# tuneinsight/lattigo

Measured on AMD Instinct MI355X. Metric: ciphertext-mul+relin ops/s, higher is better.
Workload: dtype u64; 1 GPU; BGV logN=15, 12 Q-limbs [55,45x11] + 3 P-limbs [55x3], T=65537: ct x ct MulRelin (tensor + gadget product + ModDown), inputs resident in HBM; batch_per_gpu=256, logN=15, L=12, alpha=3, beta=4, parallelism=1 independent replicas, ciphertext-sharded

## Files before the change

### lattigo_amd/csrc/kernels.hip

```cpp
#include "kernels.h"

#include <atomic>
#include <cstdio>
#include <cstdlib>
#include <type_traits>
#include <mutex>
#include <unordered_map>
#include <vector>

namespace he {

namespace {
struct ProfRec { int id; hipEvent_t e0, e1; double bytes; };
struct ProfState { std::vector<ProfRec> recs; };
std::mutex g_prof_mu;
std::atomic<int> g_prof_active{0};
std::unordered_map<hipStream_t, ProfState> g_prof;
std::vector<hipEvent_t> g_prof_pool;
hipEvent_t prof_event_locked() {
    if (!g_prof_pool.empty()) { hipEvent_t e = g_prof_pool.back(); g_prof_pool.pop_back(); return e; }
    hipEvent_t e;
    (void)hipEventCreate(&e);
    return e;
}
// ... 177 lines not shown
    const uint64_t *tw;
    const double *twd;
    int N;
    int a;
    int flags;
    int scale;
    LimbTab tab;
    int epi;
    const uint64_t *epi_y, *epi_w;
    size_t epi_y_bs, epi_w_bs;
    uint64_t epi_s[kMaxLimbs];
    int zsplit;
    int epi2;
    uint64_t *out2;
    size_t out2_bs;
    const uint64_t *epi_y2, *epi_w2;
    size_t epi_y2_bs, epi_w2_bs;
    int epi_tensor;
    const uint64_t *ta0, *ta1, *tb0, *tb1;
    size_t ta0_bs, ta1_bs, tb0_bs, tb1_bs;
    uint64_t epi_ts[kMaxLimbs];
    uint64_t io_s[kMaxLimbs];
    int epi_y_f64;
    int epi_y_reduce;
    int nbatch, iters;
    int nbatch_prof = 0;
    int tprod = 0;
    unsigned sc_ginv = 0;
    int sc_logN = 0;
    const size_t *in_tab = nullptr;
    int cb = 0;
    const size_t *out_tab = nullptr, *out2_tab = nullptr, *epi_w_tab = nullptr, *epi_w2_tab = nullptr;
    const size_t *ta0_tab = nullptr, *ta1_tab = nullptr, *tb0_tab = nullptr, *tb1_tab = nullptr;
    const size_t *epi_y_tab = nullptr, *epi_y2_tab = nullptr;
};

__device__ __forceinline__ int lds_phys(int e) { return e + (e >> 4); }

__device__ __forceinline__ void wave_lds_sync() {
    __builtin_amdgcn_fence(__ATOMIC_RELEASE, "wavefront");
    __builtin_amdgcn_wave_barrier();
    __builtin_amdgcn_fence(__ATOMIC_ACQUIRE, "wavefront");
}
__device__ __forceinline__ void rows_sync(int sh) {
    if (sh <= 6) wave_lds_sync();
    else __syncthreads();
}
template <int T>
__device__ __forceinline__ int nat_e(int k, int tau) {
    constexpr int CH = T >= 64 ? 64 : T;
    return (tau / CH) * (16 * CH) + k * CH + (tau % CH);
}

int ntt_row_bits(int n) {
    return n <= 12 ? n : (n <= 15 ? 12 : 13);
}

template <int G4, bool INV, bool NC>
__device__ __forceinline__ void rows_round(uint64_t (&x)[16], const uint64_t *__restrict__ tw, int rowtw, int s0, int hi0,
                                           int tau, int sh, uint64_t q, uint64_t twoq, uint64_t qinv, const ModConst &mc,
                                           bool scale_last) {
    constexpr int g = G4, G = 1 << g, W = 16 / G;
    if constexpr (!INV) {
#pragma unroll
        for (int u = 0; u < g; u++) {
            const int d = 1 << (g - 1 - u);
#pragma unroll
            for (int w = 0; w < W; w++) {
                const int hi = (W == 1) ? hi0 : ((tau * W + w) >> sh);
                const int base = (rowtw << (s0 + u)) + (hi << u);
#pragma unroll
                for (int k = 0; k < G; k++) {
                    if (k & d) continue;
                    const uint64_t wv = tw[base + (k >> (g - u))];
                    if constexpr (NC) bfly_fwd_nc<true>(x[w * G + k], x[w * G + k + d], wv, q, qinv);
                    else bfly_fwd<true>(x[w * G + k], x[w * G + k + d], wv, q, twoq, qinv);
                }
            }
        }
    } else {
#pragma unroll
        for (int u = g - 1; u >= 0; u--) {
            const int d = 1 << (g - 1 - u);
            const bool last = scale_last && u == 0;
#pragma unroll
            for (int w = 0; w < W; w++) {
                const int hi = (W == 1) ? hi0 : ((tau * W + w) >> sh);
                const int base = (rowtw << (s0 + u)) + (hi << u);
#pragma unroll
                for (int k = 0; k < G; k++) {
                    if (k & d) continue;
                    const uint64_t wv = tw[base + (k >> (g - u))];
                    if (last) bfly_inv_scaled(x[w * G + k], x[w * G + k + d], mred(wv, mc.ninv, q, qinv), mc.ninv, q, twoq, qinv);
                    else bfly_inv(x[w * G + k], x[w * G + k + d], wv, q, twoq, qinv);
                }
            }
        }
    }
}

__device__ __forceinline__ void rows_tw16(uint64_t (&t)[15], const uint64_t *__restrict__ tw, int rowtw, int s0, int hi0) {
#pragma unroll
    for (int u = 0; u < 4; u++) {
        const int base = (rowtw << (s0 + u)) + (hi0 << u);
#pragma unroll
        for (int j = 0; j < (1 << u); j++) t[(1 << u) - 1 + j] = tw[base + j];
// ... 760 lines not shown
template <int LOGB>
__device__ __forceinline__ void mac_final_xfer(double (&x)[16], double *lds, int tau, bool store) {
    if constexpr (LOGB % 4 == 0) rows_lds_xfer_f64<LOGB, 4>(x, lds, tau, LOGB - 4, 0, store);
    else rows_lds_xfer_f64<LOGB, LOGB % 4>(x, lds, tau, LOGB - LOGB % 4, 0, store);
}
typedef __attribute__((address_space(3))) void *he_lds_ptr;
__device__ __forceinline__ unsigned lds_byte_addr(const void *p) { return (unsigned)(uintptr_t)(he_lds_ptr)p; }
__device__ __forceinline__ void glds16(const void *gsrc, unsigned lds_dst) {
    unsigned keep;
    asm volatile("s_mov_b32 %0, m0\n\ts_mov_b32 m0, %2\n\ts_nop 0\n\tglobal_load_lds_dwordx4 %1, off nt\n\ts_mov_b32 m0, %0"
                 : "=&s"(keep) : "v"(gsrc), "s"(lds_dst) : "memory");
}
struct MacEpiK {
    const uint64_t *ext; size_t ext_bs;
    uint64_t *out0, *out1; size_t out0_bs, out1_bs;
    const uint64_t *w0, *w1; size_t w0_bs, w1_bs;
    const uint64_t *ta0, *ta1, *tb0, *tb1; size_t ta0_bs, ta1_bs, tb0_bs, tb1_bs;
    int ext_f64, tensor, has_w0, has_w1;
    double sp[kMaxLimbs], tsp[kMaxLimbs];
    const size_t *etab;
    unsigned etab_rows;
    unsigned sc_ginv;
    int sc_logN;
    int gs_accum;
};
enum { ME_OUT0 = 0, ME_OUT1, ME_W0, ME_W1, ME_TA0, ME_TA1, ME_TB0, ME_TB1 };
__device__ __forceinline__ size_t meoff(const MacEpiK &e, int which, size_t bs, size_t z, unsigned nbatch) {
    const unsigned row = (e.etab_rows >> (4 * which)) & 0xFu;
    return (e.etab && row != 0xFu) ? (size_t)ldc(reinterpret_cast<const uint64_t *>(e.etab), (size_t)row * nbatch + z) : z * bs;
}
struct NttMacDmaArgs {
    NttMacKArgs k;
    MacEpiK e;
    unsigned nbatch, nitems;
    uint64_t limb_info[kMaxLimbs];
};
#ifdef HE_MAC_STAMPS
#ifndef HE_MAC_STAMP_ITEM
#define HE_MAC_STAMP_ITEM 10
#endif
#define MAC_STAMP2(i) do { __builtin_amdgcn_sched_barrier(0); if (t_cur == HE_MAC_STAMP_ITEM && g < 512u && (threadIdx.x & 63u) == 0) g_mac_stamps[((g * 4 + (threadIdx.x >> 6)) * 64) + (i)] = __builtin_amdgcn_s_memtime(); __builtin_amdgcn_sched_barrier(0); } while (0)
#else
#define MAC_STAMP2(i) do {} while (0)
#endif
template <int LOGB, bool QF64, bool EPI = false, bool SCAT = false, bool TEN = false>
__global__ void __launch_bounds__((1 << LOGB) / 16, 2) ntt_mac_f64_dma_kernel(NttMacDmaArgs AA) {
    static_assert(LOGB == 12 || LOGB == 13, "production row sizes only");
    constexpr int N2 = 1 << LOGB;
    constexpr int T = N2 / 16;
    constexpr int GREM = LOGB % 4;
    const NttMacKArgs &A = AA.k;
    __shared__ double lds[N2 + N2 / 16];
    __shared__ double pbuf[N2];
    __shared__ double tw1s[16 * 15];

    const unsigned tau = threadIdx.x, lane = tau & 63u;
    const unsigned wv = (unsigned)__builtin_amdgcn_readfirstlane((int)(tau >> 6));
    const unsigned G = gridDim.x, g = blockIdx.x;
    const bool xcd = ((G | AA.nitems) & 7u) == 0;
    const unsigned span = xcd ? AA.nitems >> 3 : AA.nitems, stride = xcd ? G >> 3 : G;
    const unsigned first = xcd ? g >> 3 : g, base = xcd ? (g & 7u) * span : 0u;
    auto item_of = [&](unsigned t) -> unsigned { const unsigned i = first + t * stride; return i < span ? base + i : ~0u; };

    struct Item {
        size_t bz, rowoff;
        int ql, rowtw, out_limb, mi, l;
        bool isP;
        double q, qi;
        const double *tw, *kbase;
    };
    auto decode = [&](unsigned w) -> Item {
        Item it;
        it.bz = w % AA.nbatch;
        const int l = (int)((w / AA.nbatch) % (unsigned)A.m.nlimbs);
        const int row = (int)(w / (AA.nbatch * (unsigned)A.m.nlimbs));
        const uint64_t info = AA.limb_info[l];
        it.l = l;
        const int mi = (int)(info & 0xff);
        it.mi = mi;
        const uint64_t *mcw = reinterpret_cast<const uint64_t *>(A.mc + mi);
        it.q = (double)ldc(mcw, 0); it.qi = __longlong_as_double((long long)ldc(mcw, 8));
        it.tw = A.twd + (size_t)mi * A.N;
        it.rowtw = (1 << A.a) + row;
        it.rowoff = (size_t)row * N2;
        it.kbase = A.keyd + (size_t)((info >> 8) & 0xff) * A.N + it.rowoff;
        it.ql = (int)((info >> 16) & 0xff);
        it.out_limb = (int)((info >> 24) & 0xff);
        it.isP = ((info >> 32) & 0xff) != 0;
        return it;
    };
    auto own_digit = [&](const Item &it, int d) -> bool {
        return A.m.own_alpha > 0 && !it.isP && it.ql >= d * A.m.own_alpha && it.ql < (d + 1) * A.m.own_alpha;
    };
    const int nd = A.m.beta + (EPI ? 2 : 0);
    auto digit_src = [&](const Item &it, int d) -> const uint64_t * {
        if (EPI && d >= A.m.beta)
            return AA.e.ext + ((size_t)(d - A.m.beta) * AA.nbatch + it.bz) * AA.e.ext_bs + (size_t)it.ql * A.N + it.rowoff;
        return own_digit(it, d) ? A.own + voff(A.own_tab, A.own_bs, it.bz) + (size_t)it.ql * A.N + it.rowoff
                                : A.dec + it.bz * A.dec_bs + (size_t)d * A.m.dec_dstride + (size_t)it.ql * A.N + it.rowoff;
    };
    const unsigned pw_addr = lds_byte_addr(pbuf) + wv * 8192u;
    auto dma_digit = [&](const uint64_t *src, unsigned lane) {
        const uint64_t *gp = src + ((lane >> 5) * T + 64u * wv + 2u * (lane & 31u));
#pragma unroll
        for (int j = 0; j < 8; j++) glds16(gp + (size_t)j * 2 * T, pw_addr + (unsigned)j * 1024u);
    };

    unsigned t = 0;
    unsigned w = item_of(0);
    if (w == ~0u) return;
    Item cur = decode(w);
    dma_digit(digit_src(cur, 0), lane);
    for (;;) {
        const unsigned t_cur = t; (void)t_cur;
        MAC_STAMP2(0);
        double acc0[16], acc1[16];
#pragma unroll
        for (int k = 0; k < 16; k++) { acc0[k] = 0.0; acc1[k] = 0.0; }
        const double q = cur.q, qi = cur.qi;
        if (tau < 240u) {
            const unsigned hi = tau / 15u, idx = tau - hi * 15u, u = 31u - (unsigned)__builtin_clz(idx + 1u), j = idx + 1u - (1u << u);
            tw1s[tau] = cur.tw[((unsigned)cur.rowtw << (4 + u)) + (hi << u) + j];
        }
        bool more = false;
        auto round0 = [&](double (&x)[16]) {
            double t0[15];
#pragma unroll
            for (int u = 0; u < 4; u++)
#pragma unroll
                for (int j = 0; j < (1 << u); j++) t0[(1 << u) - 1 + j] = ldcd(cur.tw, (size_t)(((unsigned)cur.rowtw << u) + j));
            rows_round16_f64<false>(x, t0, q, qi);
        };
        auto round1 = [&](double (&x)[16], unsigned tau) {
            rows_lds_xfer_f64<LOGB, 4>(x, lds, tau, 4, LOGB - 8, false);
            {
                double t1[15];
                const double *tp = tw1s + (tau >> (LOGB - 8)) * 15u;
#pragma unroll
                for (int i = 0; i < 15; i++) t1[i] = tp[i];
                rows_round16_f64<false>(x, t1, q, qi);
            }
            rows_lds_xfer_f64<LOGB, 4>(x, lds, tau, 4, LOGB - 8, true);
            rows_sync(LOGB - 8);
            rows_lds_xfer_f64<LOGB, 4>(x, lds, tau, 8, LOGB - 12, false);
        };
        auto transform = [&](int nk, double (&x)[16], unsigned tau, unsigned lane, const uint64_t *nsrc, const double *k0p,
                             const double *k1p, double (&kk0)[16], double (&kk1)[16]) {
            double t2[15];
            rows_tw16_f64(t2, cur.tw, cur.rowtw, 8, tau >> (LOGB - 12));
            __builtin_amdgcn_sched_barrier(0);
            asm volatile("s_waitcnt lgkmcnt(0)" ::: "memory");
            if (nsrc) dma_digit(nsrc, lane);
            __builtin_amdgcn_sched_barrier(0);
            round0(x);
            __syncthreads();
            rows_lds_xfer_f64<LOGB, 4>(x, lds, tau, 0, LOGB - 4, true);
            __syncthreads();
            round1(x, tau);
            __builtin_amdgcn_sched_barrier(0);
            if (nk >= 1) {
#pragma unroll
                for (int k = 0; k < 16; k++) kk0[k] = k0p[(unsigned)(k * T)];
            }
            __builtin_amdgcn_sched_barrier(0);
            rows_round16_f64<false>(x, t2, q, qi);
            __builtin_amdgcn_sched_barrier(0);
            if (nk >= 2) {
#pragma unroll
                for (int k = 0; k < 16; k++) kk1[k] = k1p[(unsigned)(k * T)];
            }
            __builtin_amdgcn_sched_barrier(0);
            if constexpr (GREM > 0) {
                rows_lds_xfer_f64<LOGB, 4>(x, lds, tau, 8, LOGB - 12, true);
                rows_sync(LOGB - 12);
                rows_lds_xfer_f64<LOGB, GREM>(x, lds, tau, 12, 0, false);
                rows_round_f64<GREM, false>(x, cur.tw, cur.rowtw, 12, 0, tau, 0, q, qi);
            }
        };
        auto next_src = [&](int d) -> const uint64_t * {
            if (d + 1 < nd) return digit_src(cur, d + 1);
            w = item_of(++t);
            more = w != ~0u;
            return more ? digit_src(decode(w), 0) : nullptr;
        };
        for (int d = 0; d < A.m.beta; d++) {
            const bool is_own = own_digit(cur, d);
            unsigned tau_d = threadIdx.x;
            asm volatile("" : "+v"(tau_d));
            const unsigned tau = tau_d, lane = tau & 63u;
            const double *pw = pbuf + wv * 1024u + lane;
            MAC_STAMP2(1 + d * 12 + 0);
            asm volatile("s_waitcnt vmcnt(0)" ::: "memory");
            uint64_t xi[16];
#pragma unroll
            for (int k = 0; k < 16; k++) xi[k] = (uint64_t)__double_as_longlong(pw[k * 64]);
            double x[16];
            if (is_own && A.m.own_reduce) {
#pragma unroll
                for (int k = 0; k < 16; k++) xi[k] = bred_add_lazy(xi[k], ldc(reinterpret_cast<const uint64_t *>(A.mc + cur.mi), 0), ldc(reinterpret_cast<const uint64_t *>(A.mc + cur.mi), 2));
            }
            if (A.m.dec_f64 && !is_own) {
#pragma unroll
                for (int k = 0; k < 16; k++) x[k] = __longlong_as_double((long long)xi[k]);
            } else {
#pragma unroll
                for (int k = 0; k < 16; k++) x[k] = u52_to_f64(xi[k]);
            }
            MAC_STAMP2(1 + d * 12 + 1);
            const uint64_t *nsrc = next_src(d);
            const double *k0p = cur.kbase + (size_t)d * A.m.key_dstride + tau, *k1p = k0p + A.m.key_kstride;
            double kk0[16], kk1[16];
            if (!is_own) {
                transform(2, x, tau, lane, nsrc, k0p, k1p, kk0, kk1);
            } else {
                asm volatile("s_waitcnt lgkmcnt(0)" ::: "memory");
                if (nsrc) dma_digit(nsrc, lane);
                __builtin_amdgcn_sched_barrier(0);
#pragma unroll
                for (int k = 0; k < 16; k++) kk0[k] = k0p[(unsigned)(k * T)];
#pragma unroll
                for (int k = 0; k < 16; k++) kk1[k] = k1p[(unsigned)(k * T)];
                __builtin_amdgcn_sched_barrier(0);
                __syncthreads();
                rows_lds_xfer_f64<LOGB, 4>(x, lds, tau, 0, LOGB - 4, true);
                __syncthreads();
                mac_final_xfer<LOGB>(x, lds, tau, false);
            }
            MAC_STAMP2(1 + d * 12 + 8);
#pragma unroll
            for (int k = 0; k < 16; k++) acc0[k] += modmul_f64(x[k], kk0[k], q, qi);
            MAC_STAMP2(1 + d * 12 + 9);
#pragma unroll
            for (int k = 0; k < 16; k++) acc1[k] += modmul_f64(x[k], kk1[k], q, qi);
            MAC_STAMP2(1 + d * 12 + 10);
        }
        if constexpr (EPI && TEN && LOGB == 12) {
            unsigned tau_d = threadIdx.x;
            asm volatile("" : "+v"(tau_d));
            const unsigned tau = tau_d, lane = tau & 63u;
            const double *pw = pbuf + wv * 1024u + lane;
            MAC_STAMP2(48);
            asm volatile("s_waitcnt vmcnt(0)" ::: "memory");
            double xA[16], xB[16];
            uint64_t wB[16];
#pragma unroll
            for (int k = 0; k < 16; k++) xA[k] = pw[k * 64];
            const uint64_t *srcB = digit_src(cur, A.m.beta + 1) + tau;
            const uint64_t *nsrc = next_src(A.m.beta + 1);
#pragma unroll
            for (int k = 0; k < 16; k++) wB[k] = ldnt(&srcB[(unsigned)(k * T)]);
            double t2[15];
            rows_tw16_f64(t2, cur.tw, cur.rowtw, 8, tau);
            __builtin_amdgcn_sched_barrier(0);
            asm volatile("s_waitcnt lgkmcnt(0)" ::: "memory");
            if (nsrc) dma_digit(nsrc, lane);
            __builtin_amdgcn_sched_barrier(0);
            if (!AA.e.ext_f64) {
#pragma unroll
                for (int k = 0; k < 16; k++) xA[k] = u52_to_f64((uint64_t)__double_as_longlong(xA[k]));
            }
            MAC_STAMP2(49);
            const size_t off = (size_t)cur.out_limb * A.N + cur.rowoff + tau;
            uint64_t *op0 = AA.e.out0 + meoff(AA.e, ME_OUT0, AA.e.out0_bs, cur.bz, AA.nbatch) + off;
            uint64_t *op1 = AA.e.out1 + meoff(AA.e, ME_OUT1, AA.e.out1_bs, cur.bz, AA.nbatch) + off;
            const double sp = AA.e.sp[cur.l];
            const uint64_t *mcw = reinterpret_cast<const uint64_t *>(A.mc + cur.mi);
            const uint64_t qu = ldc(mcw, 0);
            uint64_t r0[16], r1[16], r2[16], r3[16];
            round0(xA);
            __syncthreads();
            rows_lds_xfer_f64<LOGB, 4>(xA, lds, tau, 0, LOGB - 4, true);
            if (AA.e.ext_f64) {
#pragma unroll
                for (int k = 0; k < 16; k++) xB[k] = __longlong_as_double((long long)wB[k]);
            } else {
#pragma unroll
                for (int k = 0; k < 16; k++) xB[k] = u52_to_f64(wB[k]);
            }
            round0(xB);
            __syncthreads();
            MAC_STAMP2(50);
            round1(xA, tau);
            __syncthreads();
            rows_lds_xfer_f64<LOGB, 4>(xB, lds, tau, 0, LOGB - 4, true);
            MAC_STAMP2(51);
            __builtin_amdgcn_sched_barrier(0);
            {
                const uint64_t *pa0 = AA.e.ta0 + meoff(AA.e, ME_TA0, AA.e.ta0_bs, cur.bz, AA.nbatch) + off;
                const uint64_t *pb0 = AA.e.tb0 + meoff(AA.e, ME_TB0, AA.e.tb0_bs, cur.bz, AA.nbatch) + off;
#pragma unroll
                for (int k = 0; k < 16; k++) { r0[k] = pa0[(unsigned)(k * T)]; r1[k] = pb0[(unsigned)(k * T)]; }
            }
            __builtin_amdgcn_sched_barrier(0);
            rows_round16_f64<false>(xA, t2, q, qi);
#pragma unroll
            for (int k = 0; k < 16; k++) xA[k] -= reduce_f64(acc0[k], q, qi);
            __syncthreads();
            MAC_STAMP2(52);
            round1(xB, tau);
            mac_final_xfer<LOGB>(xA, lds, tau, true);
            MAC_STAMP2(53);
            rows_round16_f64<false>(xB, t2, q, qi);
#pragma unroll
            for (int k = 0; k < 16; k++) xB[k] -= reduce_f64(acc1[k], q, qi);
            __builtin_amdgcn_sched_barrier(0);
            {
                const uint64_t *pa1 = AA.e.ta1 + meoff(AA.e, ME_TA1, AA.e.ta1_bs, cur.bz, AA.nbatch) + off;
                const uint64_t *pb1 = AA.e.tb1 + meoff(AA.e, ME_TB1, AA.e.tb1_bs, cur.bz, AA.nbatch) + off;
#pragma unroll
                for (int k = 0; k < 16; k++) { r2[k] = pa1[(unsigned)(k * T)]; r3[k] = pb1[(unsigned)(k * T)]; }
            }
            __builtin_amdgcn_sched_barrier(0);
            __syncthreads();
            MAC_STAMP2(54);
#pragma unroll
            for (int k = 0; k < 16; k++) xA[k] = lds[lds_phys(k * T + tau)];
            __syncthreads();
            mac_final_xfer<LOGB>(xB, lds, tau, true);
            MAC_STAMP2(55);
            auto cvtb = [&](uint64_t (&w)[16], double (&dd)[16]) {
                const uint64_t twoq_u = qu << 1, brc0 = ldc(mcw, 2);
                bool big = false;
#pragma unroll
                for (int k = 0; k < 16; k++) big = big || w[k] >= twoq_u;
                if (__any(big)) {
#pragma unroll
                    for (int k = 0; k < 16; k++) w[k] = bred_add_lazy(w[k], qu, brc0);
                }
#pragma unroll
                for (int k = 0; k < 16; k++) dd[k] = u52_to_f64(w[k]);
            };
            const double tsp = AA.e.tsp[cur.l];
            double u[16], v[16];
            cvtb(r0, u); cvtb(r1, v);
#pragma unroll
            for (int k = 0; k < 16; k++) {
                const double tt = modmul_f64(modmul_f64(u[k], v[k], q, qi), tsp, q, qi) + modmul_f64(xA[k], sp, q, qi);
                stnt(&op0[(unsigned)(k * T)], canon_f64(tt, q, qi));
            }
            __builtin_amdgcn_sched_barrier(0);
            __syncthreads();
            MAC_STAMP2(56);
#pragma unroll
            for (int k = 0; k < 16; k++) xB[k] = lds[lds_phys(k * T + tau)];
            double u2[16], v2[16];
            cvtb(r2, u2); cvtb(r3, v2);
#pragma unroll
            for (int k = 0; k < 16; k++) {
                const double wv = modmul_f64(u[k], v2[k], q, qi) + modmul_f64(u2[k], v[k], q, qi);
                const double tt = modmul_f64(wv, tsp, q, qi) + modmul_f64(xB[k], sp, q, qi);
                stnt(&op1[(unsigned)(k * T)], canon_f64(tt, q, qi));
            }
            MAC_STAMP2(57);
        } else if constexpr (EPI) {
            auto ext_pass = [&](auto cc) __attribute__((always_inline)) {
                const int c = cc;
                unsigned tau_d = threadIdx.x;
                asm volatile("" : "+v"(tau_d));
                const unsigned tau = tau_d, lane = tau & 63u;
                const double *pw = pbuf + wv * 1024u + lane;
                MAC_STAMP2(48 + c * 4 + 0);
                asm volatile("s_waitcnt vmcnt(0)" ::: "memory");
                double x[16];
                if (AA.e.ext_f64) {
#pragma unroll
                    for (int k = 0; k < 16; k++) x[k] = pw[k * 64];
                } else {
#pragma unroll
                    for (int k = 0; k < 16; k++) x[k] = u52_to_f64((uint64_t)__double_as_longlong(pw[k * 64]));
                }
                const uint64_t *nsrc = next_src(A.m.beta + c);
                const bool second = c != 0;
                const size_t off = (size_t)cur.out_limb * A.N + cur.rowoff + tau;
                uint64_t *op = (second ? AA.e.out1 + meoff(AA.e, ME_OUT1, AA.e.out1_bs, cur.bz, AA.nbatch) : AA.e.out0 + meoff(AA.e, ME_OUT0, AA.e.out0_bs, cur.bz, AA.nbatch)) + off;
                const double sp = AA.e.sp[cur.l];
                const uint64_t *mcw = reinterpret_cast<const uint64_t *>(A.mc + cur.mi);
                const uint64_t qu = ldc(mcw, 0);
                const bool tensor = LOGB == 13 && AA.e.tensor != 0;
                const bool addw = !tensor && (second ? AA.e.has_w1 : AA.e.has_w0) != 0;
                double kd0[16], kd1[16];
                MAC_STAMP2(48 + c * 4 + 1);
                constexpr bool prefetch = LOGB == 12;
                const uint64_t *pa0 = nullptr, *pa1 = nullptr, *pb0 = nullptr, *pb1 = nullptr, *wp = nullptr;
                if (tensor) {
                    pa0 = AA.e.ta0 + meoff(AA.e, ME_TA0, AA.e.ta0_bs, cur.bz, AA.nbatch) + off; pa1 = AA.e.ta1 + meoff(AA.e, ME_TA1, AA.e.ta1_bs, cur.bz, AA.nbatch) + off;
                    pb0 = AA.e.tb0 + meoff(AA.e, ME_TB0, AA.e.tb0_bs, cur.bz, AA.nbatch) + off; pb1 = AA.e.tb1 + meoff(AA.e, ME_TB1, AA.e.tb1_bs, cur.bz, AA.nbatch) + off;
                } else if (addw) {
                    wp = (second ? AA.e.w1 + meoff(AA.e, ME_W1, AA.e.w1_bs, cur.bz, AA.nbatch) : AA.e.w0 + meoff(AA.e, ME_W0, AA.e.w0_bs, cur.bz, AA.nbatch)) + off;
                }
                constexpr int NB = 4;
                uint64_t A0[NB], A1[NB], A2[NB], A3[NB];
                if constexpr (prefetch) transform(addw ? 1 : 0, x, tau, lane, nsrc, reinterpret_cast<const double *>(wp), nullptr, kd0, kd1);
                else transform(0, x, tau, lane, nsrc, nullptr, nullptr, kd0, kd1);
#pragma unroll
                for (int k = 0; k < 16; k++) x[k] -= reduce_f64(acc0[k], q, qi);
                mac_final_xfer<LOGB>(x, lds, tau, true);
                __syncthreads();
#pragma unroll
                for (int k = 0; k < 16; k++) x[k] = lds[lds_phys(k * T + tau)];
                MAC_STAMP2(48 + c * 4 + 2);
                if (tensor) {
                    const double tsp = AA.e.tsp[cur.l];
                    const uint64_t twoq_u = qu << 1, brc0 = ldc(mcw, 2);
                    auto cvtb = [&](uint64_t (&w)[NB], double (&dd)[NB]) {
                        bool big = false;
#pragma unroll
                        for (int k = 0; k < NB; k++) big = big || w[k] >= twoq_u;
                        if (__any(big)) {
#pragma unroll
                            for (int k = 0; k < NB; k++) w[k] = bred_add_lazy(w[k], qu, brc0);
                        }
#pragma unroll
                        for (int k = 0; k < NB; k++) dd[k] = u52_to_f64(w[k]);
                    };
                    auto issue = [&](auto hc, uint64_t (&r0)[NB], uint64_t (&r1)[NB], uint64_t (&r2)[NB], uint64_t (&r3)[NB]) {
                        constexpr int h = decltype(hc)::value;
#pragma unroll
                        for (int k = 0; k < NB; k++) { const unsigned e = (unsigned)((NB * h + k) * T); r0[k] = pa0[e]; r1[k] = pb0[e]; }
                        if (second) {
#pragma unroll
                            for (int k = 0; k < NB; k++) { const unsigned e = (unsigned)((NB * h + k) * T); r2[k] = pa1[e]; r3[k] = pb1[e]; }
                        }
                        __builtin_amdgcn_sched_barrier(0);
                    };
                    auto finish = [&](auto hc, uint64_t (&r0)[NB], uint64_t (&r1)[NB], uint64_t (&r2)[NB], uint64_t (&r3)[NB]) {
                        constexpr int h = decltype(hc)::value;
                        double u[NB], v[NB], u2[NB], v2[NB], wv[NB];
                        cvtb(r0, u); cvtb(r1, v);
                        if (second) {
                            cvtb(r2, u2); cvtb(r3, v2);
#pragma unroll
                            for (int k = 0; k < NB; k++) wv[k] = modmul_f64(u[k], v2[k], q, qi) + modmul_f64(u2[k], v[k], q, qi);
                        } else {
#pragma unroll
                            for (int k = 0; k < NB; k++) wv[k] = modmul_f64(u[k], v[k], q, qi);
                        }
#pragma unroll
                        for (int k = 0; k < NB; k++) {
                            const int i = NB * h + k;
                            const double tt = modmul_f64(wv[k], tsp, q, qi) + modmul_f64(x[i], sp, q, qi);
                            stnt(&op[(unsigned)(i * T)], canon_f64(tt, q, qi));
                        }
                        __builtin_amdgcn_sched_barrier(0);
                    };
#define HE_H(n) std::integral_constant<int, n>{}
                    issue(HE_H(0), A0, A1, A2, A3); finish(HE_H(0), A0, A1, A2, A3);
                    issue(HE_H(1), A0, A1, A2, A3); finish(HE_H(1), A0, A1, A2, A3);
                    issue(HE_H(2), A0, A1, A2, A3); finish(HE_H(2), A0, A1, A2, A3);
                    issue(HE_H(3), A0, A1, A2, A3); finish(HE_H(3), A0, A1, A2, A3);
#undef HE_H
                } else if (addw) {
                    uint64_t wv[16];
                    if constexpr (prefetch) {
#pragma unroll
                        for (int k = 0; k < 16; k++) wv[k] = (uint64_t)__double_as_longlong(kd0[k]);
                    } else {
#pragma unroll
                        for (int k = 0; k < 16; k++) wv[k] = ldnt(&wp[(unsigned)(k * T)]);
                    }
#pragma unroll
                    for (int k = 0; k < 16; k++) {
                        const uint64_t v = canon_f64(modmul_f64(x[k], sp, q, qi), q, qi);
                        uint64_t *dp = &op[(unsigned)(k * T)];
                        if constexpr (SCAT) dp = op - (cur.rowoff + tau) + auto_dest((unsigned)(cur.rowoff + tau) + (unsigned)(k * T), AA.e.sc_ginv, AA.e.sc_logN);
                        stnt(dp, cred(wv[k] + v, qu));
                    }
                } else {
#pragma unroll
                    for (int k = 0; k < 16; k++) {
                        uint64_t *dp = &op[(unsigned)(k * T)];
                        if constexpr (SCAT) dp = op - (cur.rowoff + tau) + auto_dest((unsigned)(cur.rowoff + tau) + (unsigned)(k * T), AA.e.sc_ginv, AA.e.sc_logN);
                        stnt(dp, canon_f64(modmul_f64(x[k], sp, q, qi), q, qi));
                    }
                }
                MAC_STAMP2(48 + c * 4 + 3);
#pragma unroll
                for (int k = 0; k < 16; k++) acc0[k] = acc1[k];
            };
            if constexpr (LOGB == 12) {
                ext_pass(std::integral_constant<int, 0>{});
                ext_pass(std::integral_constant<int, 1>{});
            } else {
#pragma unroll 1
                for (int c = 0; c < 2; c++) ext_pass(c);
            }
        }
        const int ol = cur.out_limb;
        uint64_t *o0 = nullptr, *o1 = nullptr;
        unsigned tau_t = threadIdx.x;
        asm volatile("" : "+v"(tau_t));
        const unsigned tau = tau_t;
        if constexpr (!EPI) {
            o0 = (cur.isP ? A.o0P + voff(A.oP0_tab, A.oP0_bs, cur.bz) : A.o0Q + voff(A.oQ0_tab, A.oQ0_bs, cur.bz)) + (size_t)ol * A.N + cur.rowoff + tau;
            o1 = (cur.isP ? A.o1P + voff(A.oP1_tab, A.oP1_bs, cur.bz) : A.o1Q + voff(A.oQ1_tab, A.oQ1_bs, cur.bz)) + (size_t)ol * A.N + cur.rowoff + tau;
        }
        [[maybe_unused]] uint64_t gs_av[16], gs_p0[16], gs_p1[16];
        [[maybe_unused]] const uint64_t *gs_ap = nullptr;
        if constexpr (!EPI && SCAT) {
            __builtin_amdgcn_sched_barrier(0);
            const size_t src = cur.rowoff + tau;
            if (AA.e.has_w0) gs_ap = (cur.isP ? AA.e.w1 + meoff(AA.e, ME_W1, AA.e.w1_bs, cur.bz, AA.nbatch) : AA.e.w0 + meoff(AA.e, ME_W0, AA.e.w0_bs, cur.bz, AA.nbatch)) + (size_t)ol * A.N + src;
            if (gs_ap) {
#pragma unroll
                for (int k = 0; k < 16; k++) gs_av[k] = ldnt(&gs_ap[(unsigned)(k * T)]);
            }
            if (AA.e.gs_accum) {
                const uint64_t *b0p = o0 - src;
#pragma unroll
                for (int k = 0; k < 16; k++) gs_p0[k] = b0p[auto_dest((unsigned)src + (unsigned)(k * T), AA.e.sc_ginv, AA.e.sc_logN)];
            }
            __builtin_amdgcn_sched_barrier(0);
        }
        if constexpr (!EPI) {
            auto to_natural = [&](double (&a)[16]) {
                mac_final_xfer<LOGB>(a, lds, tau, true);
                __syncthreads();
#pragma unroll
                for (int k = 0; k < 16; k++) a[k] = lds[lds_phys(k * T + tau)];
            };
            to_natural(acc0);
            if constexpr (SCAT) {
                const uint64_t qu = ldc(reinterpret_cast<const uint64_t *>(A.mc + cur.mi), 0);
                const size_t src = cur.rowoff + tau;
                uint64_t *b0p = o0 - src;
                const uint64_t *b1p = o1 - src;
                const bool accum = AA.e.gs_accum != 0;
                if (accum) {
#pragma unroll
                    for (int k = 0; k < 16; k++) gs_p1[k] = b1p[auto_dest((unsigned)src + (unsigned)(k * T), AA.e.sc_ginv, AA.e.sc_logN)];
                }
                __builtin_amdgcn_sched_barrier(0);
#pragma unroll
                for (int k = 0; k < 16; k++) {
                    uint64_t v0 = canon_f64(acc0[k], q, qi);
                    if (gs_ap) v0 = cred(v0 + gs_av[k], qu);
                    if (accum) v0 += gs_p0[k];
                    stnt(&b0p[auto_dest((unsigned)src + (unsigned)(k * T), AA.e.sc_ginv, AA.e.sc_logN)], v0);
                }
            }
            __syncthreads();
            to_natural(acc1);
        }
        if constexpr (EPI) {
            (void)o0; (void)o1; (void)ol;
        } else if constexpr (SCAT) {
            const size_t src = cur.rowoff + tau;
            uint64_t *b1p = o1 - src;
            const bool accum = AA.e.gs_accum != 0;
#pragma unroll
            for (int k = 0; k < 16; k++) {
                uint64_t v1 = canon_f64(acc1[k], q, qi);
                if (accum) v1 += gs_p1[k];
                stnt(&b1p[auto_dest((unsigned)src + (unsigned)(k * T), AA.e.sc_ginv, AA.e.sc_logN)], v1);
            }
        } else if constexpr (QF64) {
            double *d0 = reinterpret_cast<double *>(o0), *d1 = reinterpret_cast<double *>(o1);
#pragma unroll
            for (int k = 0; k < 16; k++) {
                stnt(&d0[(unsigned)(k * T)], reduce_f64(acc0[k], q, qi));
                stnt(&d1[(unsigned)(k * T)], reduce_f64(acc1[k], q, qi));
            }
        } else {
#pragma unroll
            for (int k = 0; k < 16; k++) {
                o0[(unsigned)(k * T)] = canon_f64(acc0[k], q, qi);
                o1[(unsigned)(k * T)] = canon_f64(acc1[k], q, qi);
            }
        }
        MAC_STAMP2(60);
        if (!more) break;
        cur = decode(w);
    }
}

static unsigned mac_resident_workgroups(int logb) {
    static const unsigned cus = [] {
        int dev = 0, n = 0;
        if (hipGetDevice(&dev) != hipSuccess || hipDeviceGetAttribute(&n, hipDeviceAttributeMultiprocessorCount, dev) != hipSuccess || n <= 0)
            n = 256;
        return (unsigned)n;
    }();
    return logb >= 13 ? cus : 2u * cus;
}

bool ntt_prod_in_supported(int logN) {
    const int b = ntt_row_bits(logN);
    return b == 12 || b == 13;
}
bool epilogue_scatter_supported(int logN) {
    const int b = ntt_row_bits(logN);
    return b == 12 || b == 13;
}
bool ntt_mac_epilogue_supported(int logN) {
    const int b = ntt_row_bits(logN);
    return b == 12 || b == 13;
}
bool ntt_mac_giant_supported(int logN) {
    const int b = ntt_row_bits(logN);
    return b == 12 || b == 13;
}
hipError_t launch_ntt_mac_f64(const RingDev &r, const NttMacArgs &a, View dec, View own, const double *keyd, View out0Q,
                              View out0P, View out1Q, View out1P, int batch, hipStream_t s, const NttMacEpilogue *epi,
                              const KsScatter *giant) {
    if (a.nlimbs <= 0 || batch <= 0) return hipSuccess;
    if (!r.twd_fwd || !keyd) return hipErrorInvalidValue;
    if (giant && (epi || a.q_out_f64 || !giant->ginv || !ntt_mac_giant_supported(r.logN))) return hipErrorInvalidValue;
    if (dec.tab || (epi && epi->ext.tab) || (a.q_out_f64 && !no_tab({out0Q, out1Q}))) return hipErrorInvalidValue;
    const int b = ntt_row_bits(r.logN), aa = r.logN - b;
    if (epi && !ntt_mac_epilogue_supported(r.logN)) return hipErrorInvalidValue;
    NttMacKArgs A{};
    A.dec = dec.p; A.dec_bs = dec.bstride; A.own = own.p; A.own_bs = own.bstride; A.own_tab = own.tab; A.keyd = keyd;
    A.o0Q = out0Q.p; A.o0P = out0P.p; A.o1Q = out1Q.p; A.o1P = out1P.p;
    A.oQ0_bs = out0Q.bstride; A.oP0_bs = out0P.bstride; A.oQ1_bs = out1Q.bstride; A.oP1_bs = out1P.bstride;
    A.oQ0_tab = out0Q.tab; A.oP0_tab = out0P.tab; A.oQ1_tab = out1Q.tab; A.oP1_tab = out1P.tab;
    A.mc = r.mc; A.twd = r.twd_fwd; A.N = r.N; A.a = aa; A.m = a;
    double mac_bytes = ((double)a.beta * batch + 2.0 * a.beta + 2.0 * batch) * a.nlimbs * (double)r.N * 8.0;
    if (epi) mac_bytes += (2.0 + (epi->tensor ? 4.0 : (epi->has_w0 ? 1.0 : 0.0) + (epi->has_w1 ? 1.0 : 0.0))) * batch * a.nlimbs * (double)r.N * 8.0;
    if (epi || giant || b >= 12) {
        NttMacDmaArgs D;
// ... 2627 lines not shown
```

Baseline: 44490 ctxt-mul+relin ops/s.

## Use wave-local chunked natural layout in NTT-MAC kernel, replacing block barriers

Rewrites the data layout the fused NTT-MAC kernel uses for the natural order. Each wave now owns a contiguous 1024-element chunk (nat_e/nat_phys), so output, epilogue and own-digit DMA accesses stride by 64 instead of T. Because each wave only touches its own LDS chunk, many __syncthreads calls become wave-local syncs. The stage-1 twiddle buffer is double-buffered and skipped when the beta=1 own-digit path does not need it. The risk is the correctness of the indexing: the chunked element order must match for every producer and consumer, including the scatter (auto_dest) paths.

```diff
diff --git a/lattigo_amd/csrc/kernels.hip b/lattigo_amd/csrc/kernels.hip
--- a/lattigo_amd/csrc/kernels.hip
+++ b/lattigo_amd/csrc/kernels.hip
@@ -253,6 +253,12 @@
     return (tau / CH) * (16 * CH) + k * CH + (tau % CH);
 }
 
+template <int T>
+__device__ __forceinline__ int nat_phys(int k, int tau) {
+    static_assert(T >= 64, "whole waves");
+    return lds_phys(nat_e<T>(0, tau)) + 68 * k;
+}
+
 int ntt_row_bits(int n) {
     return n <= 12 ? n : (n <= 15 ? 12 : 13);
 }
@@ -1119,7 +1125,7 @@
     const NttMacKArgs &A = AA.k;
     __shared__ double lds[N2 + N2 / 16];
     __shared__ double pbuf[N2];
-    __shared__ double tw1s[16 * 15];
+    __shared__ double tw1s[2][16 * 15];
 
     const unsigned tau = threadIdx.x, lane = tau & 63u;
     const unsigned wv = (unsigned)__builtin_amdgcn_readfirstlane((int)(tau >> 6));
@@ -1167,17 +1173,23 @@
                                 : A.dec + it.bz * A.dec_bs + (size_t)d * A.m.dec_dstride + (size_t)it.ql * A.N + it.rowoff;
     };
     const unsigned pw_addr = lds_byte_addr(pbuf) + wv * 8192u;
-    auto dma_digit = [&](const uint64_t *src, unsigned lane) {
-        const uint64_t *gp = src + ((lane >> 5) * T + 64u * wv + 2u * (lane & 31u));
-#pragma unroll
-        for (int j = 0; j < 8; j++) glds16(gp + (size_t)j * 2 * T, pw_addr + (unsigned)j * 1024u);
+    auto dma_digit = [&](const uint64_t *src, unsigned lane, bool chunk) {
+        if (chunk) {
+            const uint64_t *gp = src + (1024u * wv + 2u * lane);
+#pragma unroll
+            for (int j = 0; j < 8; j++) glds16(gp + (size_t)j * 128, pw_addr + (unsigned)j * 1024u);
+        } else {
+            const uint64_t *gp = src + ((lane >> 5) * T + 64u * wv + 2u * (lane & 31u));
+#pragma unroll
+            for (int j = 0; j < 8; j++) glds16(gp + (size_t)j * 2 * T, pw_addr + (unsigned)j * 1024u);
+        }
     };
 
-    unsigned t = 0;
+    unsigned t = 0, tw1h = 0;
     unsigned w = item_of(0);
     if (w == ~0u) return;
     Item cur = decode(w);
-    dma_digit(digit_src(cur, 0), lane);
+    dma_digit(digit_src(cur, 0), lane, own_digit(cur, 0));
     for (;;) {
         const unsigned t_cur = t; (void)t_cur;
         MAC_STAMP2(0);
@@ -1185,9 +1197,12 @@
 #pragma unroll
         for (int k = 0; k < 16; k++) { acc0[k] = 0.0; acc1[k] = 0.0; }
         const double q = cur.q, qi = cur.qi;
-        if (tau < 240u) {
-            const unsigned hi = tau / 15u, idx = tau - hi * 15u, u = 31u - (unsigned)__builtin_clz(idx + 1u), j = idx + 1u - (1u << u);
-            tw1s[tau] = cur.tw[((unsigned)cur.rowtw << (4 + u)) + (hi << u) + j];
+        if (EPI || A.m.beta > 1 || !own_digit(cur, 0)) {
+            tw1h ^= 1u;
+            if (tau < 240u) {
+                const unsigned hi = tau / 15u, idx = tau - hi * 15u, u = 31u - (unsigned)__builtin_clz(idx + 1u), j = idx + 1u - (1u << u);
+                tw1s[tw1h][tau] = cur.tw[((unsigned)cur.rowtw << (4 + u)) + (hi << u) + j];
+            }
         }
         bool more = false;
         auto round0 = [&](double (&x)[16]) {
@@ -1202,7 +1217,7 @@
             rows_lds_xfer_f64<LOGB, 4>(x, lds, tau, 4, LOGB - 8, false);
             {
                 double t1[15];
-                const double *tp = tw1s + (tau >> (LOGB - 8)) * 15u;
+                const double *tp = tw1s[tw1h] + (tau >> (LOGB - 8)) * 15u;
 #pragma unroll
                 for (int i = 0; i < 15; i++) t1[i] = tp[i];
                 rows_round16_f64<false>(x, t1, q, qi);
@@ -1211,13 +1226,14 @@
             rows_sync(LOGB - 8);
             rows_lds_xfer_f64<LOGB, 4>(x, lds, tau, 8, LOGB - 12, false);
         };
-        auto transform = [&](int nk, double (&x)[16], unsigned tau, unsigned lane, const uint64_t *nsrc, const double *k0p,
-                             const double *k1p, double (&kk0)[16], double (&kk1)[16]) {
+        auto transform = [&](int nk, auto k0s, double (&x)[16], unsigned tau, unsigned lane, const uint64_t *nsrc, bool nchunk,
+                             const double *k0p, const double *k1p, double (&kk0)[16], double (&kk1)[16]) {
+            constexpr unsigned K0S = decltype(k0s)::value;
             double t2[15];
             rows_tw16_f64(t2, cur.tw, cur.rowtw, 8, tau >> (LOGB - 12));
             __builtin_amdgcn_sched_barrier(0);
             asm volatile("s_waitcnt lgkmcnt(0)" ::: "memory");
-            if (nsrc) dma_digit(nsrc, lane);
+            if (nsrc) dma_digit(nsrc, lane, nchunk);
             __builtin_amdgcn_sched_barrier(0);
             round0(x);
             __syncthreads();
@@ -1227,7 +1243,7 @@
             __builtin_amdgcn_sched_barrier(0);
             if (nk >= 1) {
 #pragma unroll
-                for (int k = 0; k < 16; k++) kk0[k] = k0p[(unsigned)(k * T)];
+                for (int k = 0; k < 16; k++) kk0[k] = k0p[(unsigned)k * K0S];
             }
             __builtin_amdgcn_sched_barrier(0);
             rows_round16_f64<false>(x, t2, q, qi);
@@ -1244,11 +1260,18 @@
                 rows_round_f64<GREM, false>(x, cur.tw, cur.rowtw, 12, 0, tau, 0, q, qi);
             }
         };
-        auto next_src = [&](int d) -> const uint64_t * {
-            if (d + 1 < nd) return digit_src(cur, d + 1);
+        auto next_src = [&](int d, bool &chunk) -> const uint64_t * {
+            if (d + 1 < nd) {
+                chunk = d + 1 < A.m.beta && own_digit(cur, d + 1);
+                return digit_src(cur, d + 1);
+            }
             w = item_of(++t);
             more = w != ~0u;
-            return more ? digit_src(decode(w), 0) : nullptr;
+            chunk = false;
+            if (!more) return nullptr;
+            const Item nx = decode(w);
+            chunk = own_digit(nx, 0);
+            return digit_src(nx, 0);
         };
         for (int d = 0; d < A.m.beta; d++) {
             const bool is_own = own_digit(cur, d);
@@ -1274,23 +1297,24 @@
                 for (int k = 0; k < 16; k++) x[k] = u52_to_f64(xi[k]);
             }
             MAC_STAMP2(1 + d * 12 + 1);
-            const uint64_t *nsrc = next_src(d);
+            bool nchunk;
+            const uint64_t *nsrc = next_src(d, nchunk);
             const double *k0p = cur.kbase + (size_t)d * A.m.key_dstride + tau, *k1p = k0p + A.m.key_kstride;
             double kk0[16], kk1[16];
             if (!is_own) {
-                transform(2, x, tau, lane, nsrc, k0p, k1p, kk0, kk1);
+                transform(2, std::integral_constant<unsigned, (unsigned)T>{}, x, tau, lane, nsrc, nchunk, k0p, k1p, kk0, kk1);
             } else {
                 asm volatile("s_waitcnt lgkmcnt(0)" ::: "memory");
-                if (nsrc) dma_digit(nsrc, lane);
+                if (nsrc) dma_digit(nsrc, lane, nchunk);
                 __builtin_amdgcn_sched_barrier(0);
 #pragma unroll
                 for (int k = 0; k < 16; k++) kk0[k] = k0p[(unsigned)(k * T)];
 #pragma unroll
                 for (int k = 0; k < 16; k++) kk1[k] = k1p[(unsigned)(k * T)];
                 __builtin_amdgcn_sched_barrier(0);
-                __syncthreads();
-                rows_lds_xfer_f64<LOGB, 4>(x, lds, tau, 0, LOGB - 4, true);
-                __syncthreads();
+#pragma unroll
+                for (int k = 0; k < 16; k++) lds[nat_phys<T>(k, tau)] = x[k];
+                wave_lds_sync();
                 mac_final_xfer<LOGB>(x, lds, tau, false);
             }
             MAC_STAMP2(1 + d * 12 + 8);
@@ -1313,21 +1337,22 @@
 #pragma unroll
             for (int k = 0; k < 16; k++) xA[k] = pw[k * 64];
             const uint64_t *srcB = digit_src(cur, A.m.beta + 1) + tau;
-            const uint64_t *nsrc = next_src(A.m.beta + 1);
+            bool nchunk;
+            const uint64_t *nsrc = next_src(A.m.beta + 1, nchunk);
 #pragma unroll
             for (int k = 0; k < 16; k++) wB[k] = ldnt(&srcB[(unsigned)(k * T)]);
             double t2[15];
             rows_tw16_f64(t2, cur.tw, cur.rowtw, 8, tau);
             __builtin_amdgcn_sched_barrier(0);
             asm volatile("s_waitcnt lgkmcnt(0)" ::: "memory");
-            if (nsrc) dma_digit(nsrc, lane);
+            if (nsrc) dma_digit(nsrc, lane, nchunk);
             __builtin_amdgcn_sched_barrier(0);
             if (!AA.e.ext_f64) {
 #pragma unroll
                 for (int k = 0; k < 16; k++) xA[k] = u52_to_f64((uint64_t)__double_as_longlong(xA[k]));
             }
             MAC_STAMP2(49);
-            const size_t off = (size_t)cur.out_limb * A.N + cur.rowoff + tau;
+            const size_t off = (size_t)cur.out_limb * A.N + cur.rowoff + (unsigned)nat_e<T>(0, tau);
             uint64_t *op0 = AA.e.out0 + meoff(AA.e, ME_OUT0, AA.e.out0_bs, cur.bz, AA.nbatch) + off;
             uint64_t *op1 = AA.e.out1 + meoff(AA.e, ME_OUT1, AA.e.out1_bs, cur.bz, AA.nbatch) + off;
             const double sp = AA.e.sp[cur.l];
@@ -1356,7 +1381,7 @@
                 const uint64_t *pa0 = AA.e.ta0 + meoff(AA.e, ME_TA0, AA.e.ta0_bs, cur.bz, AA.nbatch) + off;
                 const uint64_t *pb0 = AA.e.tb0 + meoff(AA.e, ME_TB0, AA.e.tb0_bs, cur.bz, AA.nbatch) + off;
 #pragma unroll
-                for (int k = 0; k < 16; k++) { r0[k] = pa0[(unsigned)(k * T)]; r1[k] = pb0[(unsigned)(k * T)]; }
+                for (int k = 0; k < 16; k++) { r0[k] = pa0[(unsigned)(k * 64)]; r1[k] = pb0[(unsigned)(k * 64)]; }
             }
             __builtin_amdgcn_sched_barrier(0);
             rows_round16_f64<false>(xA, t2, q, qi);
@@ -1375,14 +1400,14 @@
                 const uint64_t *pa1 = AA.e.ta1 + meoff(AA.e, ME_TA1, AA.e.ta1_bs, cur.bz, AA.nbatch) + off;
                 const uint64_t *pb1 = AA.e.tb1 + meoff(AA.e, ME_TB1, AA.e.tb1_bs, cur.bz, AA.nbatch) + off;
 #pragma unroll
-                for (int k = 0; k < 16; k++) { r2[k] = pa1[(unsigned)(k * T)]; r3[k] = pb1[(unsigned)(k * T)]; }
+                for (int k = 0; k < 16; k++) { r2[k] = pa1[(unsigned)(k * 64)]; r3[k] = pb1[(unsigned)(k * 64)]; }
             }
             __builtin_amdgcn_sched_barrier(0);
-            __syncthreads();
+            wave_lds_sync();
             MAC_STAMP2(54);
 #pragma unroll
-            for (int k = 0; k < 16; k++) xA[k] = lds[lds_phys(k * T + tau)];
-            __syncthreads();
+            for (int k = 0; k < 16; k++) xA[k] = lds[nat_phys<T>(k, tau)];
+            wave_lds_sync();
             mac_final_xfer<LOGB>(xB, lds, tau, true);
             MAC_STAMP2(55);
             auto cvtb = [&](uint64_t (&w)[16], double (&dd)[16]) {
@@ -1403,20 +1428,20 @@
 #pragma unroll
             for (int k = 0; k < 16; k++) {
                 const double tt = modmul_f64(modmul_f64(u[k], v[k], q, qi), tsp, q, qi) + modmul_f64(xA[k], sp, q, qi);
-                stnt(&op0[(unsigned)(k * T)], canon_f64(tt, q, qi));
+                stnt(&op0[(unsigned)(k * 64)], canon_f64(tt, q, qi));
             }
             __builtin_amdgcn_sched_barrier(0);
-            __syncthreads();
+            wave_lds_sync();
             MAC_STAMP2(56);
 #pragma unroll
-            for (int k = 0; k < 16; k++) xB[k] = lds[lds_phys(k * T + tau)];
+            for (int k = 0; k < 16; k++) xB[k] = lds[nat_phys<T>(k, tau)];
             double u2[16], v2[16];
             cvtb(r2, u2); cvtb(r3, v2);
 #pragma unroll
             for (int k = 0; k < 16; k++) {
                 const double wv = modmul_f64(u[k], v2[k], q, qi) + modmul_f64(u2[k], v[k], q, qi);
                 const double tt = modmul_f64(wv, tsp, q, qi) + modmul_f64(xB[k], sp, q, qi);
-                stnt(&op1[(unsigned)(k * T)], canon_f64(tt, q, qi));
+                stnt(&op1[(unsigned)(k * 64)], canon_f64(tt, q, qi));
             }
             MAC_STAMP2(57);
         } else if constexpr (EPI) {
@@ -1436,9 +1461,11 @@
 #pragma unroll
                     for (int k = 0; k < 16; k++) x[k] = u52_to_f64((uint64_t)__double_as_longlong(pw[k * 64]));
                 }
-                const uint64_t *nsrc = next_src(A.m.beta + c);
+                bool nchunk;
+                const uint64_t *nsrc = next_src(A.m.beta + c, nchunk);
                 const bool second = c != 0;
-                const size_t off = (size_t)cur.out_limb * A.N + cur.rowoff + tau;
+                const unsigned tn = (unsigned)nat_e<T>(0, tau);
+                const size_t off = (size_t)cur.out_limb * A.N + cur.rowoff + tn;
                 uint64_t *op = (second ? AA.e.out1 + meoff(AA.e, ME_OUT1, AA.e.out1_bs, cur.bz, AA.nbatch) : AA.e.out0 + meoff(AA.e, ME_OUT0, AA.e.out0_bs, cur.bz, AA.nbatch)) + off;
                 const double sp = AA.e.sp[cur.l];
                 const uint64_t *mcw = reinterpret_cast<const uint64_t *>(A.mc + cur.mi);
@@ -1457,14 +1484,15 @@
                 }
                 constexpr int NB = 4;
                 uint64_t A0[NB], A1[NB], A2[NB], A3[NB];
-                if constexpr (prefetch) transform(addw ? 1 : 0, x, tau, lane, nsrc, reinterpret_cast<const double *>(wp), nullptr, kd0, kd1);
-                else transform(0, x, tau, lane, nsrc, nullptr, nullptr, kd0, kd1);
+                constexpr std::integral_constant<unsigned, 64u> ws{};
+                if constexpr (prefetch) transform(addw ? 1 : 0, ws, x, tau, lane, nsrc, nchunk, reinterpret_cast<const double *>(wp), nullptr, kd0, kd1);
+                else transform(0, ws, x, tau, lane, nsrc, nchunk, nullptr, nullptr, kd0, kd1);
 #pragma unroll
                 for (int k = 0; k < 16; k++) x[k] -= reduce_f64(acc0[k], q, qi);
                 mac_final_xfer<LOGB>(x, lds, tau, true);
-                __syncthreads();
-#pragma unroll
-                for (int k = 0; k < 16; k++) x[k] = lds[lds_phys(k * T + tau)];
+                wave_lds_sync();
+#pragma unroll
+                for (int k = 0; k < 16; k++) x[k] = lds[nat_phys<T>(k, tau)];
                 MAC_STAMP2(48 + c * 4 + 2);
                 if (tensor) {
                     const double tsp = AA.e.tsp[cur.l];
@@ -1483,10 +1511,10 @@
                     auto issue = [&](auto hc, uint64_t (&r0)[NB], uint64_t (&r1)[NB], uint64_t (&r2)[NB], uint64_t (&r3)[NB]) {
                         constexpr int h = decltype(hc)::value;
 #pragma unroll
-                        for (int k = 0; k < NB; k++) { const unsigned e = (unsigned)((NB * h + k) * T); r0[k] = pa0[e]; r1[k] = pb0[e]; }
+                        for (int k = 0; k < NB; k++) { const unsigned e = (unsigned)((NB * h + k) * 64); r0[k] = pa0[e]; r1[k] = pb0[e]; }
                         if (second) {
 #pragma unroll
-                            for (int k = 0; k < NB; k++) { const unsigned e = (unsigned)((NB * h + k) * T); r2[k] = pa1[e]; r3[k] = pb1[e]; }
+                            for (int k = 0; k < NB; k++) { const unsigned e = (unsigned)((NB * h + k) * 64); r2[k] = pa1[e]; r3[k] = pb1[e]; }
                         }
                         __builtin_amdgcn_sched_barrier(0);
                     };
@@ -1506,7 +1534,7 @@
                         for (int k = 0; k < NB; k++) {
                             const int i = NB * h + k;
                             const double tt = modmul_f64(wv[k], tsp, q, qi) + modmul_f64(x[i], sp, q, qi);
-                            stnt(&op[(unsigned)(i * T)], canon_f64(tt, q, qi));
+                            stnt(&op[(unsigned)(i * 64)], canon_f64(tt, q, qi));
                         }
                         __builtin_amdgcn_sched_barrier(0);
                     };
@@ -1523,20 +1551,20 @@
                         for (int k = 0; k < 16; k++) wv[k] = (uint64_t)__double_as_longlong(kd0[k]);
                     } else {
 #pragma unroll
-                        for (int k = 0; k < 16; k++) wv[k] = ldnt(&wp[(unsigned)(k * T)]);
+                        for (int k = 0; k < 16; k++) wv[k] = ldnt(&wp[(unsigned)(k * 64)]);
                     }
 #pragma unroll
                     for (int k = 0; k < 16; k++) {
                         const uint64_t v = canon_f64(modmul_f64(x[k], sp, q, qi), q, qi);
-                        uint64_t *dp = &op[(unsigned)(k * T)];
-                        if constexpr (SCAT) dp = op - (cur.rowoff + tau) + auto_dest((unsigned)(cur.rowoff + tau) + (unsigned)(k * T), AA.e.sc_ginv, AA.e.sc_logN);
+                        uint64_t *dp = &op[(unsigned)(k * 64)];
+                        if constexpr (SCAT) dp = op - (cur.rowoff + tn) + auto_dest((unsigned)(cur.rowoff + tn) + (unsigned)(k * 64), AA.e.sc_ginv, AA.e.sc_logN);
                         stnt(dp, cred(wv[k] + v, qu));
                     }
                 } else {
 #pragma unroll
                     for (int k = 0; k < 16; k++) {
-                        uint64_t *dp = &op[(unsigned)(k * T)];
-                        if constexpr (SCAT) dp = op - (cur.rowoff + tau) + auto_dest((unsigned)(cur.rowoff + tau) + (unsigned)(k * T), AA.e.sc_ginv, AA.e.sc_logN);
+                        uint64_t *dp = &op[(unsigned)(k * 64)];
+                        if constexpr (SCAT) dp = op - (cur.rowoff + tn) + auto_dest((unsigned)(cur.rowoff + tn) + (unsigned)(k * 64), AA.e.sc_ginv, AA.e.sc_logN);
                         stnt(dp, canon_f64(modmul_f64(x[k], sp, q, qi), q, qi));
                     }
                 }
@@ -1557,44 +1585,45 @@
         unsigned tau_t = threadIdx.x;
         asm volatile("" : "+v"(tau_t));
         const unsigned tau = tau_t;
+        [[maybe_unused]] const unsigned tn = (unsigned)nat_e<T>(0, tau);
         if constexpr (!EPI) {
-            o0 = (cur.isP ? A.o0P + voff(A.oP0_tab, A.oP0_bs, cur.bz) : A.o0Q + voff(A.oQ0_tab, A.oQ0_bs, cur.bz)) + (size_t)ol * A.N + cur.rowoff + tau;
-            o1 = (cur.isP ? A.o1P + voff(A.oP1_tab, A.oP1_bs, cur.bz) : A.o1Q + voff(A.oQ1_tab, A.oQ1_bs, cur.bz)) + (size_t)ol * A.N + cur.rowoff + tau;
+            o0 = (cur.isP ? A.o0P + voff(A.oP0_tab, A.oP0_bs, cur.bz) : A.o0Q + voff(A.oQ0_tab, A.oQ0_bs, cur.bz)) + (size_t)ol * A.N + cur.rowoff + tn;
+            o1 = (cur.isP ? A.o1P + voff(A.oP1_tab, A.oP1_bs, cur.bz) : A.o1Q + voff(A.oQ1_tab, A.oQ1_bs, cur.bz)) + (size_t)ol * A.N + cur.rowoff + tn;
         }
         [[maybe_unused]] uint64_t gs_av[16], gs_p0[16], gs_p1[16];
         [[maybe_unused]] const uint64_t *gs_ap = nullptr;
         if constexpr (!EPI && SCAT) {
             __builtin_amdgcn_sched_barrier(0);
-            const size_t src = cur.rowoff + tau;
+            const size_t src = cur.rowoff + tn;
             if (AA.e.has_w0) gs_ap = (cur.isP ? AA.e.w1 + meoff(AA.e, ME_W1, AA.e.w1_bs, cur.bz, AA.nbatch) : AA.e.w0 + meoff(AA.e, ME_W0, AA.e.w0_bs, cur.bz, AA.nbatch)) + (size_t)ol * A.N + src;
             if (gs_ap) {
 #pragma unroll
-                for (int k = 0; k < 16; k++) gs_av[k] = ldnt(&gs_ap[(unsigned)(k * T)]);
+                for (int k = 0; k < 16; k++) gs_av[k] = ldnt(&gs_ap[(unsigned)(k * 64)]);
             }
             if (AA.e.gs_accum) {
                 const uint64_t *b0p = o0 - src;
 #pragma unroll
-                for (int k = 0; k < 16; k++) gs_p0[k] = b0p[auto_dest((unsigned)src + (unsigned)(k * T), AA.e.sc_ginv, AA.e.sc_logN)];
+                for (int k = 0; k < 16; k++) gs_p0[k] = b0p[auto_dest((unsigned)src + (unsigned)(k * 64), AA.e.sc_ginv, AA.e.sc_logN)];
             }
             __builtin_amdgcn_sched_barrier(0);
         }
         if constexpr (!EPI) {
             auto to_natural = [&](double (&a)[16]) {
                 mac_final_xfer<LOGB>(a, lds, tau, true);
-                __syncthreads();
-#pragma unroll
-                for (int k = 0; k < 16; k++) a[k] = lds[lds_phys(k * T + tau)];
+                wave_lds_sync();
+#pragma unroll
+                for (int k = 0; k < 16; k++) a[k] = lds[nat_phys<T>(k, tau)];
             };
             to_natural(acc0);
             if constexpr (SCAT) {
                 const uint64_t qu = ldc(reinterpret_cast<const uint64_t *>(A.mc + cur.mi), 0);
-                const size_t src = cur.rowoff + tau;
+                const size_t src = cur.rowoff + tn;
                 uint64_t *b0p = o0 - src;
                 const uint64_t *b1p = o1 - src;
                 const bool accum = AA.e.gs_accum != 0;
                 if (accum) {
 #pragma unroll
-                    for (int k = 0; k < 16; k++) gs_p1[k] = b1p[auto_dest((unsigned)src + (unsigned)(k * T), AA.e.sc_ginv, AA.e.sc_logN)];
+                    for (int k = 0; k < 16; k++) gs_p1[k] = b1p[auto_dest((unsigned)src + (unsigned)(k * 64), AA.e.sc_ginv, AA.e.sc_logN)];
                 }
                 __builtin_amdgcn_sched_barrier(0);
 #pragma unroll
@@ -1602,36 +1631,36 @@
                     uint64_t v0 = canon_f64(acc0[k], q, qi);
                     if (gs_ap) v0 = cred(v0 + gs_av[k], qu);
                     if (accum) v0 += gs_p0[k];
-                    stnt(&b0p[auto_dest((unsigned)src + (unsigned)(k * T), AA.e.sc_ginv, AA.e.sc_logN)], v0);
-                }
-            }
-            __syncthreads();
+                    stnt(&b0p[auto_dest((unsigned)src + (unsigned)(k * 64), AA.e.sc_ginv, AA.e.sc_logN)], v0);
+                }
+            }
+            wave_lds_sync();
             to_natural(acc1);
         }
         if constexpr (EPI) {
             (void)o0; (void)o1; (void)ol;
         } else if constexpr (SCAT) {
-            const size_t src = cur.rowoff + tau;
+            const size_t src = cur.rowoff + tn;
             uint64_t *b1p = o1 - src;
             const bool accum = AA.e.gs_accum != 0;
 #pragma unroll
             for (int k = 0; k < 16; k++) {
                 uint64_t v1 = canon_f64(acc1[k], q, qi);
                 if (accum) v1 += gs_p1[k];
-                stnt(&b1p[auto_dest((unsigned)src + (unsigned)(k * T), AA.e.sc_ginv, AA.e.sc_logN)], v1);
+                stnt(&b1p[auto_dest((unsigned)src + (unsigned)(k * 64), AA.e.sc_ginv, AA.e.sc_logN)], v1);
             }
         } else if constexpr (QF64) {
             double *d0 = reinterpret_cast<double *>(o0), *d1 = reinterpret_cast<double *>(o1);
 #pragma unroll
             for (int k = 0; k < 16; k++) {
-                stnt(&d0[(unsigned)(k * T)], reduce_f64(acc0[k], q, qi));
-                stnt(&d1[(unsigned)(k * T)], reduce_f64(acc1[k], q, qi));
+                stnt(&d0[(unsigned)(k * 64)], reduce_f64(acc0[k], q, qi));
+                stnt(&d1[(unsigned)(k * 64)], reduce_f64(acc1[k], q, qi));
             }
         } else {
 #pragma unroll
             for (int k = 0; k < 16; k++) {
-                o0[(unsigned)(k * T)] = canon_f64(acc0[k], q, qi);
-                o1[(unsigned)(k * T)] = canon_f64(acc1[k], q, qi);
+                o0[(unsigned)(k * 64)] = canon_f64(acc0[k], q, qi);
+                o1[(unsigned)(k * 64)] = canon_f64(acc1[k], q, qi);
             }
         }
         MAC_STAMP2(60);
```

After: 44720 ctxt-mul+relin ops/s (median of 6 runs). About the same (+0.5%).
